# cloudwego/dynamicgo

Hardware: AMD Instinct MI355X
Metric: conv/j2t GB/s JSON in + msgs/s, 64K-batch device-resident, 1→8 MI355X (higher is better)
Workload: dtype u8; 1 GPU; C2: 65536 flat baseline.Simple messages <=256 B, seed 42; global_batch=65536, msgs_per_rank=65536, thrift_bytes_rank0=6662181, flags=1, parallelism=dp1 (one batch per rank, descriptor broadcast over -), no data-path collective, inflight=2

## Files before the change

dynamicgo_amd/build.py:

```python
import hashlib
import os
import subprocess
import sys

ROOT = os.path.dirname(os.path.dirname(os.path.abspath(__file__)))
CSRC = os.path.join(ROOT, "dynamicgo_amd", "csrc")
HIPCC = os.environ.get("HIPCC", "/opt/rocm/bin/hipcc")
ARCH = os.environ.get("DG_OFFLOAD_ARCH", "gfx950")


def _run(cmd, cwd=None):
    print("+", " ".join(cmd), flush=True)
    subprocess.run(cmd, cwd=cwd, check=True)


UNITS = ("j2t_kern_wave.hip", "j2t_kern_wave5.hip", "j2t_kern_small.hip", "j2t_kern_lds.hip", "j2t_kern_glb.hip",
         "j2t_host.hip", "j2t_pipe.hip", "t2j_kern.hip", "t2j_host.hip", "j2t_kern_flat.hip",
         "tget_kern.hip", "tget_host.hip", "cut_kern.hip", "cut_host.hip", "edit_kern.hip", "edit_host.hip",
         "kids_kern.hip", "kids_host.hip", "editm_kern.hip", "editm_host.hip")
HEADERS = ("j2t_small.h", "j2t_wave.h", "j2t_machine.h", "j2t_device.h", "j2t_fast.h", "dg_tables.h", "host_internal.h",
           "t2j_device.h", "t2j_tables.h", "j2t_flat.h", "t2j_wave.h", "tget_device.h", "cut_device.h", "edit_device.h",
           "kids_device.h", "editm_device.h")


def source_hash(extra_flags=()) -> str:
    h = hashlib.sha256()
    for f in sorted(UNITS + HEADERS):
        with open(os.path.join(CSRC, f), "rb") as fh:
            h.update(f.encode() + b"\0" + fh.read())
    for f in ("dgj2t.h", "dgj2t_defs.h", "dgj2t_desc.h"):
        with open(os.path.join(ROOT, "include", f), "rb") as fh:
            h.update(f.encode() + b"\0" + fh.read())
    h.update(repr((ARCH, COMMON_FLAGS, sorted(DEFAULT_UNIT_FLAGS.items()), tuple(extra_flags))).encode())
    return h.hexdigest()[:16]


COMMON_FLAGS = ("-O3", "-std=c++17", "-fPIC", "-ffp-contract=off", "-Wno-unused-result")
_NO_LICM = ("-mllvm", "-disable-machine-licm")
DEFAULT_UNIT_FLAGS = {"j2t_kern_flat.hip": _NO_LICM, "j2t_kern_wave.hip": _NO_LICM, "j2t_kern_wave5.hip": _NO_LICM,
                      "t2j_kern.hip": _NO_LICM}
MARK = b"dgj2t-build:"


def _deps(unit: str):
    import re
    seen, todo = [], [unit]
    while todo:
        f = todo.pop()
        if f in seen:
            continue
        seen.append(f)
        p = os.path.join(CSRC, f) if os.path.exists(os.path.join(CSRC, f)) else os.path.join(ROOT, "include", f)
        with open(p) as fh:
            for inc in re.findall(r'^\s*#\s*include\s+"([^"]+)"', fh.read(), re.M):
                todo.append(os.path.basename(inc))
    return sorted(seen)


def unit_hash(unit: str, extra_flags=()) -> str:
    h = hashlib.sha256()
    for f in _deps(unit):
        p = os.path.join(CSRC, f) if os.path.exists(os.path.join(CSRC, f)) else os.path.join(ROOT, "include", f)
        with open(p, "rb") as fh:
            h.update(f.encode() + b"\0" + fh.read())
    h.update(repr((ARCH, COMMON_FLAGS, tuple(extra_flags))).encode())
    return h.hexdigest()[:16]


def embedded_hash(path: str):
    try:
        with open(path, "rb") as fh:
            data = fh.read()
    except OSError:
        return None
    k = data.find(MARK)
    if k < 0:
        return None
    return data[k + len(MARK):k + len(MARK) + 16].decode("ascii", "replace")


def build_hip(force=False, extra_flags=(), out=None, unit_flags=None):
    out = out or os.path.join(ROOT, "dynamicgo_amd", "libdgj2t.so")
    unit_flags = unit_flags or {}
    sh = source_hash(tuple(extra_flags) + tuple(sorted((u, tuple(f)) for u, f in unit_flags.items())))
    uf0 = dict(DEFAULT_UNIT_FLAGS)
    for u, f in unit_flags.items():
        uf0[u] = tuple(uf0.get(u, ())) + tuple(f)
    unit_flags = uf0
    if not force and embedded_hash(out) == sh:
        print(f"libdgj2t.so up to date (sources {sh})", flush=True)
        return out
    objdir = os.path.join(ROOT, "build", "obj")
    os.makedirs(objdir, exist_ok=True)
    common = [HIPCC, f"--offload-arch={ARCH}", *COMMON_FLAGS, *extra_flags]
    procs, objs = [], []
    for u in UNITS:
        uf = tuple(extra_flags) + tuple(unit_flags.get(u, ()))
        uh = unit_hash(u, uf) + (sh if u == "j2t_host.hip" else "")
        o = os.path.join(objdir, u.replace(".hip", "") + "_" + uh + ".o")
        objs.append(o)
        if os.path.exists(o) and not force:
            continue
        cmd = common + list(unit_flags.get(u, ())) + ([f'-DDG_SRC_HASH="{sh}"'] if u == "j2t_host.hip" else [])
        cmd = cmd + ["-c", "-o", o + ".tmp", os.path.join(CSRC, u)]
        print("+", " ".join(cmd), flush=True)
# ... 29 lines not shown
```

dynamicgo_amd/csrc/host_internal.h:

```cpp
#pragma once
#include <hip/hip_runtime.h>

#include <stdint.h>
#include <stdlib.h>

#include <algorithm>
#include <memory>
#include <mutex>
#include <vector>

#include "../../include/dgj2t.h"
#include "../../include/dgj2t_desc.h"

__attribute__((visibility("hidden"))) int set_err(int code, const char *fmt, ...);
#define HIPCHK(x)                                                                              \
    do {                                                                                       \
        hipError_t e_ = (x);                                                                   \
        if (e_ != hipSuccess) return set_err(DG_E_HIP, "%s: %s", #x, hipGetErrorString(e_));  \
    } while (0)


template <class T, hipError_t (*FREE)(void *)>
struct ArrBase {
    T *p = nullptr;
// ... 186 lines not shown
};

struct PipeBuf;
struct PipeBufDelete {
    void operator()(PipeBuf *p) const;
};

struct dg_ctx {
    int device = 0;
    Stream stream;
    int n_cu = 0;
    Knobs knobs;
    uint32_t rr = 0;
    std::mutex mu;
    const Event *kt = nullptr;
    Event fork_ev;
    std::vector<Event> side_ev;
    std::vector<Stream> side;
    SharedWs tget;
    DevArr<uint32_t> tget_list, tget_cnt_buf;
    AltCounters tget_cnt;
    StreamOrder cut;
    DevArr<uint32_t> cut_list, cut_cnt_buf;
    AltCounters cut_cnt;
    StreamOrder edit;
    DevArr<dg_tget_rec> edit_rec;
    uint64_t edit_rec_n = 0;
    StreamOrder editm;
    DevArr<dg_tget_rec> editm_rec;
    SharedWs kids;
    DevArr<uint32_t> kids_list, kids_cnt_buf;
    AltCounters kids_cnt;
    DevArr<uint64_t> kids_sums;
    SharedWs t2j_tok;
    SharedWs t2j_deep;
    PinArr<uint8_t> h_down;
    PinArr<uint8_t> h_up;
    DevArr<uint64_t> d_pack_off;
    DevArr<uint8_t> d_pack;
    DevArr<uint8_t> d_cb;
    DevArr<uint64_t> d_aux;
    DevArr<uint64_t> d_ret;
    DevArr<uint32_t> d_out_len;
    DevArr<uint64_t> d_out_off;
    DevArr<uint8_t> d_out;
    DevArr<uint64_t> d_in_off;
    DevArr<uint8_t> d_json;
    DevArr<unsigned long long> d_stats;
    DevArr<uint64_t> d_zero;
    DevArr<uint32_t> d_pending;
    std::vector<std::unique_ptr<Scratch>> scratch;
    std::mutex pipe_mu;
    PinArr<uint8_t> h_pipe_aux, h_pipe_out;
    PinArr<uint8_t> h_pipe_ovf;
    DevArr<uint64_t> d_pipe_cur;
    std::vector<std::unique_ptr<PipeBuf, PipeBufDelete>> pipe;
    ~dg_ctx()
    {
        (void)hipSetDevice(device);
        if (stream) (void)hipStreamSynchronize(stream);
    }
};

struct Entry {
    std::unique_lock<std::mutex> lk;
    hipStream_t s = nullptr;
    int rc = DG_OK;
    Entry(dg_ctx *c, bool ok, void *stream = nullptr, const char *what = "bad args")
    {
        if (!ok) {
            rc = set_err(DG_E_INVALID, "%s", what);
            return;
        }
        lk = std::unique_lock<std::mutex>(c->mu);
        const hipError_t e = hipSetDevice(c->device);
        if (e != hipSuccess) rc = set_err(DG_E_HIP, "hipSetDevice(c->device): %s", hipGetErrorString(e));
        s = stream ? (hipStream_t)stream : (hipStream_t)c->stream;
    }
};

struct dg_desc {
    dg_ctx *ctx = nullptr;
    DevArr<uint8_t> d_blob;
    size_t len = 0;
    dg_desc_hdr hdr;
    DevArr<uint8_t> d_side;
    std::vector<uint8_t> hblob;
    size_t side_len = 0;
};

struct dg_path {
    dg_ctx *ctx;
    DevArr<uint8_t> d_blob;
    dg_path_hdr hdr;
};

struct TGetBatch {
    const uint8_t *src;
    const uint64_t *in_off;
    uint64_t n;
    dg_tget_rec *rec;
    uint64_t *val_off;
    uint32_t *val_len;
    uint64_t max_len;
};

__attribute__((visibility("hidden"))) int dg_i_path_validate(const void *blob, size_t len, dg_path_hdr &h);

__attribute__((visibility("hidden"))) int tget_launch(dg_ctx *c, const dg_path *ps, uint8_t root_type,
                                                      const TGetBatch &b, hipStream_t s);

struct HMIn {
    const dg_hm_entry *tab = nullptr;
    uint32_t n_hm = 0;
    const uint8_t *bytes = nullptr;
    const dg_cb_entry *vm = nullptr;
};

struct BatchArgs {
    const uint8_t *src = nullptr;
    const uint64_t *in_off = nullptr;
    uint64_t n = 0, flags = 0;
    uint8_t *out = nullptr;
    const uint64_t *out_off = nullptr;
    uint32_t *out_len = nullptr;
    uint64_t *ret = nullptr;
    uint32_t *pending = nullptr;
    uint64_t max_len = 0;
    HMIn hm;
    uint64_t *aux = nullptr;
};

struct HostOut {
    uint8_t *out;
    uint64_t out_cap;
    uint64_t *out_off, *out_need;
};

struct PackChain {
    const uint64_t *base_in = nullptr;
    uint64_t dst_cap = 0;
    int base_mod16 = 0;
    uint64_t *ret_dst = nullptr, *cur_out = nullptr, *ovf_out = nullptr;
    hipEvent_t pack_after = nullptr;
};

__attribute__((visibility("hidden"))) void dg_i_scratch_release(dg_ctx *c, const hipStream_t *s, int n);

__attribute__((visibility("hidden"))) int scratch_for(dg_ctx *c, hipStream_t s, Scratch **out);

__attribute__((visibility("hidden"))) int dg_i_convert_pack(dg_ctx *c, const dg_desc *d, uint32_t root,
                                                            const BatchArgs &b, uint8_t *packed, uint64_t *pack_off,
                                                            hipStream_t s, const PackChain &ch);

__attribute__((visibility("hidden"))) int dg_i_pack_scan(dg_ctx *c, hipStream_t s, const BatchArgs &b, uint8_t *d_dst,
                                                         uint64_t *d_dst_off);
```

dynamicgo_amd/csrc/j2t_flat.h:

```cpp
#pragma once
#include "j2t_small.h"

namespace dg {

constexpr uint32_t FL_G = 4;
#ifndef DG_FL_WAVES
#define DG_FL_WAVES 4
#endif
constexpr uint32_t FL_WAVES = DG_FL_WAVES;
#ifndef DG_FL_FPW
#define DG_FL_FPW 2
#endif
constexpr uint32_t FL_FPW = DG_FL_FPW;
constexpr uint32_t FL_SLOTS = FL_FPW * FL_WAVES;
constexpr uint32_t FL_MPB = 64;
constexpr uint32_t FL_LW = 9;
constexpr uint32_t FL_MAXLEN = 256;
constexpr uint32_t FL_SLOTW = FL_MAXLEN / 8;
constexpr uint32_t FL_STAGEW = FL_MPB * FL_SLOTW;
constexpr uint32_t FL_SLACKW = FL_G * FL_LW + 2;
constexpr uint32_t FL_MAXF = 24;
constexpr uint32_t FL_DESC = 16 * 1024;
#ifndef DG_FL_INLINE
#define DG_FL_INLINE 8
#endif
#ifndef DG_FL_CHUNK
#define DG_FL_CHUNK 32
#endif
constexpr uint32_t FL_INLINE = DG_FL_INLINE;
constexpr uint32_t FL_CHUNK = DG_FL_CHUNK;
constexpr uint32_t FL_MAXTASK = 320;
constexpr uint32_t FL_KEYS = 32;
constexpr uint32_t FL_NESC = 8;
#ifndef DG_FL_WPE
#define DG_FL_WPE 4
#endif

#ifndef DG_FL_DEFER_NUM
#define DG_FL_DEFER_NUM 0
#endif
#ifndef DG_FL_PERM
#define DG_FL_PERM 0
#endif
#ifndef DG_FL_REMAP
#define DG_FL_REMAP 1
#endif

#ifdef DG_FLPROF_G
#define FLG_ARG , uint64_t *flg
#define FLG_PASS , flg
#define FLG(k)                                             \
    do {                                                   \
        const uint64_t now_ = __builtin_amdgcn_s_memtime(); \
        flg[k] += now_ - flg[7];                           \
        flg[7] = now_;                                     \
    } while (0)
#else
#define FLG_ARG
#define FLG_PASS
#define FLG(k)
#endif
DGI uint32_t fl_slot(uint32_t w, uint32_t h)
{
    return DG_FL_PERM == 1 ? (h & 1 ? (h + 1) * FL_WAVES - 1 - w : h * FL_WAVES + w) : w + h * FL_WAVES;
}

#define DG_DPP(v, ctrl) ((uint32_t)__builtin_amdgcn_update_dpp(0, (int)(v), (ctrl), 0xF, 0xF, false))
DGI uint32_t g4_incl_sum(uint32_t v, uint32_t g)
{
    uint32_t t = DG_DPP(v, 0x111);
    v += g >= 1 ? t : 0u;
    t = DG_DPP(v, 0x112);
    v += g >= 2 ? t : 0u;
    return v;
}
DGI uint32_t g4_sum(uint32_t v)
{
    v += DG_DPP(v, 0xB1);
    v += DG_DPP(v, 0x4E);
    return v;
}
DGI uint32_t g4_next(uint32_t v, uint32_t g)
{
    const uint32_t t = DG_DPP(v, 0x101);
    return g < 3 ? t : 0u;
}

DGI uint32_t eq32(uint32_t w, uint32_t cc) { return zb32(w ^ cc); }

struct LSrc {
    typedef int32_t idx;
    const __attribute__((address_space(3))) uint64_t *w8;
    int32_t off0;
    int32_t n;
    DGI void init(const __attribute__((address_space(3))) uint64_t *words, int32_t off, int32_t len)
    {
        w8 = words;
        off0 = off;
        n = len;
    }
    DGI uint8_t raw(int32_t i) const
    {
        return ((const __attribute__((address_space(3))) uint8_t *)w8)[off0 + i];
    }
    DGI uint8_t at(int32_t i) const { return (uint32_t)i < (uint32_t)n ? raw(i) : 0; }
    DGI uint64_t get8(int32_t i) const
    {
        const uint32_t b = (uint32_t)(off0 + i), k = b >> 3, sh = (b & 7) << 3;
        const uint64_t lo = w8[k], hi = w8[k + 1];
        return (lo >> sh) | ((hi << 1) << (63 - sh));
    }
    DGI LSrc sub(int32_t s0, int32_t len) const
    {
        LSrc r;
        r.init(w8, off0 + s0, len);
        return r;
// ... 314 lines not shown
DGI bool body_b64(S &src, uint32_t s0, uint32_t n, bool last, O &o)
{
    typedef typename S::idx SI;
    uint32_t ip = 0;
    const uint32_t full = last && n >= 4 ? n - 4 : n;
    for (; ip + 8 <= full; ip += 8) {
        uint64_t v;
        if (!b64_8(src.get8((SI)(s0 + ip)), v)) return false;
        o.wle(v, 6);
    }
    for (; ip < full; ip += 4) {
        uint32_t v;
        if (!b64_4((uint32_t)src.get8((SI)(s0 + ip)), v)) return false;
        o.wle(v, 3);
    }
    if (last && n >= 4) {
        uint32_t w = (uint32_t)src.get8((SI)(s0 + ip));
        const uint32_t c2 = (w >> 16) & 0xFF, c3 = w >> 24;
        if (c2 == '=' && c3 != '=') return false;
        const uint32_t keep = c3 == '=' ? (c2 == '=' ? 1u : 2u) : 3u;
        if (c3 == '=') w = (w & 0x00FFFFFFu) | ((uint32_t)'A' << 24);
        if (c2 == '=') w = (w & 0xFF00FFFFu) | ((uint32_t)'A' << 16);
        uint32_t v;
        if (!b64_4(w, v)) return false;
        o.wle(v, keep);
    }
    return true;
}

template <class S, class O>
DGI uint32_t flat_write(S &src, const FField &F, const FastTabs &tb, O &o, lds_esc *E, uint32_t ne)
{
    typedef typename S::idx SI;
    if (F.kind == FV_NONE) return 1;
    bool isint = F.isint;
    int64_t iv = F.iv;
    double dv = F.dv;
    if (F.kind == FV_NUM && F.defer) {
        SI qq = (SI)F.s0;
        if (!fast_vnumber(src, qq, tb, iv, dv, isint) || (uint32_t)qq != F.s0 + F.nb) return 0;
    }
    o.wle((uint32_t)F.tt | ((uint32_t)__builtin_bswap16(F.id) << 8), 3);
    switch (F.kind) {
    case FV_BOOL: o.w8((uint8_t)iv); return 1;
    case FV_NUM:
        if (F.i16q) {
            emit_number(o, DG_T_I16, isint, iv, dv);
            emit_number(o, DG_T_BYTE, isint, iv, dv);
            return 1;
        }
        return emit_number(o, F.tt, isint, iv, dv) ? 1u : 0u;
    case FV_NUMSTR:
    case FV_STR:
        o.w32(F.kind == FV_NUMSTR ? F.nb : F.size - 7);
        if (F.esc) {
            uint32_t cur = F.s0;
            const uint32_t end = F.s0 + F.nb;
            for (uint32_t it = 0; it < FL_NESC; it++) {
                uint32_t best = 0xFFFFFFFFu;
                for (uint32_t e = 0; e < ne; e++) {
                    const uint32_t x = E[e], p = esc_pos(x);
                    if (p >= cur && p < end && p < esc_pos(best)) best = x;
                }
                if (best == 0xFFFFFFFFu) break;
                const uint32_t p = esc_pos(best);
                body_copy(src, cur, p - cur, o);
                o.wle(esc_utf8(best), esc_out(best));
                cur = p + esc_in(best);
            }
            body_copy(src, cur, end - cur, o);
            return 1;
        }
        if (F.nb > FL_INLINE) return 2;
        body_copy(src, F.s0, F.nb, o);
        return 1;
    default:
        o.w32(F.size - 7);
        if (F.nb > FL_INLINE) return 2;
        return body_b64(src, F.s0, F.nb, true, o) ? 1u : 0u;
    }
}

struct FlatParams {
    const uint8_t *blob;
    dg_desc_hdr hdr;
    uint32_t *bail_count;
    uint32_t *bail_list;
    uint32_t wrap;
    uint32_t wrap_inner;
    uint64_t wrap_ok;
};

#ifdef DG_FLPROF
#define FLP_DECL uint64_t flp_t = __builtin_amdgcn_s_memtime(); uint64_t flp[8] = {0, 0, 0, 0, 0, 0, 0, 0};
#define FLP(k)                                              \
    do {                                                    \
        const uint64_t now_ = __builtin_amdgcn_s_memtime(); \
        flp[k] += now_ - flp_t;                             \
        flp_t = now_;                                       \
    } while (0)
#define FLP_END()                                                                        \
    do {                                                                                 \
        if ((threadIdx.x & 63) == 0 && (blockIdx.x & 31) == 0)                           \
            for (int k_ = 0; k_ < 8; k_++) atomicAdd(&P.stats[2 + k_], (unsigned long long)flp[k_]); \
    } while (0)
#else
#define FLP_DECL
#define FLP(k)
#define FLP_END()
#endif
#ifdef DG_FLPROF_F
#define FLF_DECL uint64_t flf[12] = {0, 0, 0, 0, 0, 0, 0, 0, 0, 0, 0, 0};
#define FLF_T0() const uint64_t flf_t0 = __builtin_amdgcn_s_memtime()
#define FLF_ADD(k) do { if ((k) < 12) flf[k] += __builtin_amdgcn_s_memtime() - flf_t0; } while (0)
#define FLF_END()                                                                         \
    do {                                                                                  \
        if ((threadIdx.x & 63) == 0 && (blockIdx.x & 31) == 0)                            \
            for (int k_ = 0; k_ < 12; k_++) atomicAdd(&P.stats[2 + k_], (unsigned long long)flf[k_]); \
    } while (0)
#else
#define FLF_DECL
#define FLF_T0()
#define FLF_ADD(k)
#define FLF_END()
#endif

struct FlatLds {
    uint64_t in[FL_STAGEW + FL_SLACKW];
    uint64_t task[FL_MAXTASK];
    uint64_t oa[FL_MPB];
    uint32_t cap[FL_MPB];
    uint32_t ok[FL_MPB];
    uint32_t n[FL_MPB];
    uint32_t lw[FL_MPB];
    uint32_t oc[FL_MPB];
    uint32_t nfq[FL_MPB];
    uint32_t plo[FL_MPB], phi[FL_MPB];
    uint32_t big[FL_MPB];
    uint32_t nbytes[FL_MPB];
    uint32_t wid[FL_MPB];
    uint32_t nesc[FL_MPB];
    uint32_t esc[FL_MPB * FL_NESC];
    uint64_t kw[2 * FL_KEYS];
    uint32_t km[FL_KEYS];
    uint32_t fkm[FL_SLOTS];
    uint32_t sep[FL_MAXF * FL_MPB];
    uint16_t col[FL_MAXF * FL_MPB];
    uint16_t size[2 * FL_SLOTS * FL_MPB];
    uint32_t fseen[FL_MPB];
    uint32_t rounds, ntask, tgrab, noremap;
    uint8_t *a_out;
    uint64_t *a_ret;
    uint32_t *a_out_len, *a_bail_count, *a_bail_list;
    uint32_t a_nb, a_wrap;
    uint64_t p10u[20];
    double p10d[23];
    uint64_t pw[EL_WN];
};

template <int V>
__global__ __launch_bounds__(64 * FL_WAVES) __attribute__((amdgpu_waves_per_eu(DG_FL_WPE))) void j2t_flat_kernel(
    Params P, FlatParams S)
{
    __shared__ __attribute__((aligned(16))) FlatLds L;
    extern __shared__ __attribute__((aligned(16))) uint64_t s_fdesc[];
    FLP_DECL
    FLF_DECL
    const uint32_t tid = threadIdx.x, lane = tid & 63, wave = tid >> 6;
    const uint64_t b0 = (uint64_t)blockIdx.x * FL_MPB;
    const uint64_t b1 = b0 + FL_MPB < P.n ? b0 + FL_MPB : P.n;

    const uint64_t lo = P.in_off[b0], hi = P.in_off[b1];
    const uint64_t base = lo & ~15ull;
    const bool staged = hi - base <= (uint64_t)FL_STAGEW * 8;
    if (staged) {
        const uint4 *gs = (const uint4 *)(P.json + base);
        uint4 *ls = (uint4 *)L.in;
        const uint32_t nw = (uint32_t)((hi - base + 15) >> 4);
        constexpr uint32_t NT = 64 * FL_WAVES;
        static_assert(FL_STAGEW * 8 / 16 <= 4 * NT, "four 16-byte loads per thread cover the stage");
        if (nw) {
            const uint32_t l = nw - 1;
            const uint4 v0 = gs[min(tid, l)], v1 = gs[min(tid + NT, l)], v2 = gs[min(tid + 2 * NT, l)],
                        v3 = gs[min(tid + 3 * NT, l)];
            if (tid < nw) ls[tid] = v0;
            if (tid + NT < nw) ls[tid + NT] = v1;
            if (tid + 2 * NT < nw) ls[tid + 2 * NT] = v2;
            if (tid + 3 * NT < nw) ls[tid + 3 * NT] = v3;
        }
    }
    {
        const uint4 *gd = (const uint4 *)S.blob;
        uint4 *ld = (uint4 *)s_fdesc;
        for (uint32_t k = tid; k < (S.hdr.total_len + 15) / 16; k += 64 * FL_WAVES) ld[k] = gd[k];
    }
    if (tid < 20) {
        uint64_t v = 1;
        for (uint32_t k = 0; k < tid; k++) v *= 10;
        L.p10u[tid] = v;
    }
    if (tid < 23) L.p10d[tid] = P10[tid];
    el_window_fill(L.pw, tid);
    if (tid == 0) {
        L.rounds = 0;
        L.ntask = 0;
        L.tgrab = 0;
        L.noremap = 0;
        L.a_out = P.out;
        L.a_ret = P.ret;
        L.a_out_len = P.out_len;
        L.a_bail_count = S.bail_count;
        L.a_bail_list = S.bail_list;
        L.a_nb = (uint32_t)(b1 - b0);
        L.a_wrap = S.wrap;
    }
    if (tid < FL_MPB) {
        uint32_t ok = 0, n = 0, lw = 0, big = 0, cap = 0;
        uint64_t oa = 0;
        const uint64_t i = b0 + tid;
        if (i < b1) {
            const uint64_t a = P.in_off[i], b = P.in_off[i + 1];
            const uint64_t n64 = b - a;
            oa = P.out_off[i];
            cap = (uint32_t)min(P.out_off[i + 1] - oa, (uint64_t)0xFFFFFFFFu);
            const bool tobig = P.big_list && (n64 > P.big_max || n64 > FL_MAXLEN);
            list_big_w(P, tobig, i, n64);
            if (tobig) {
                big = 1;
            } else if (n64 > 0 && n64 <= FL_MAXLEN) {
                n = (uint32_t)n64;
                if (staged) {
                    ok = 1;
                    lw = (uint32_t)(((a - base) >> 3) << 3) | (uint32_t)(a & 7);
                } else {
                    ok = 1;
                    lw = (tid * FL_SLOTW) << 3;
                }
            }
        }
        L.ok[tid] = ok;
        L.n[tid] = n;
        L.lw[tid] = lw;
        L.big[tid] = big;
        L.oa[tid] = oa;
        L.cap[tid] = cap;
        L.plo[tid] = 0;
        L.phi[tid] = 0;
        L.oc[tid] = 0;
        L.nfq[tid] = 0;
        L.nesc[tid] = 0;
        L.fseen[tid] = 0;
    }
    if (tid < FL_SLOTS * FL_MPB / 4) ((uint32_t *)(void *)L.task)[tid] = 0xFFFFFFFFu;
    __syncthreads();
    const uint32_t g = tid & 3, m1 = tid >> 2;
    if (!staged) {
        if (tid < FL_G * FL_MPB && L.ok[m1]) {
            const uint64_t a = P.in_off[b0 + m1];
            const uint32_t nw = (L.n[m1] + 7) >> 3, sh = (uint32_t)(a & 7) << 3;
            const glb_u64 *gsrc = (const glb_u64 *)(const void *)P.json + (a >> 3);
            constexpr uint32_t NWL = FL_MAXLEN / 8 / FL_G;
            uint64_t lo[NWL], hi[NWL];
#pragma unroll
            for (uint32_t j = 0; j < NWL; j++) {
                const uint32_t w = g + FL_G * j;
                lo[j] = gsrc[min(w, nw)];
                hi[j] = gsrc[min(w + 1, nw)];
            }
#pragma unroll
            for (uint32_t j = 0; j < NWL; j++) {
                const uint32_t w = g + FL_G * j;
                if (w < nw) L.in[(L.lw[m1] >> 3) + w] = sh ? (lo[j] >> sh) | (hi[j] << (64 - sh)) : lo[j];
            }
        }
        __syncthreads();
    }
    FLP(0);
#if defined(DG_FL_STOP) && DG_FL_STOP == 9
    return;
#endif
    const auto D = desc_view<3>((const __attribute__((address_space(3))) uint8_t *)(void *)s_fdesc, S.hdr);
    const FastTabs tb{(const __attribute__((address_space(3))) uint64_t *)(void *)L.p10u, (lds_f64 *)(void *)L.p10d,
                      (const __attribute__((address_space(3))) uint64_t *)(void *)L.pw};
    const dg_type rt = ldrec(&D.T[S.wrap ? S.wrap_inner : P.root]);
    const dg_struct sd = ldrec(&D.S[rt.st]);
    const uint32_t nk = sd.name_mask + 1 <= FL_KEYS ? sd.name_mask + 1 : 0u;
    if (tid < nk) {
        const dg_name nm = ldrec(&D.N[sd.name_begin + tid]);
        uint32_t mt = 0xFF000000u;
        uint64_t w0 = 0, w1 = 0;
        if (nm.field != DG_NONE && nm.key_len <= 16) {
            const __attribute__((address_space(3))) uint64_t *pk = (decltype(&D.R[0]))(&D.P[nm.key_off]);
            w0 = nm.key_len ? pk[0] : 0ull;
            w1 = nm.key_len > 8 ? pk[1] : 0ull;
            mt = nm.field | (nm.key_len << 24);
        }
        L.km[tid] = mt;
        L.kw[2 * tid] = w0;
        L.kw[2 * tid + 1] = w1;
    }
    if (tid >= 64 && tid < 64 + FL_SLOTS) {
        const uint32_t j = tid - 64;
        uint32_t len = 0xFF;
        if (j < sd.n_fields) {
            const dg_field f = ldrec(&D.F[sd.field_begin + j]);
            if (f.flags & DG_FF_ALIAS_SELF) len = f.key_len;
        }
        L.fkm[j] = len;
    }
    if (S.wrap) {
        if (tid < FL_MPB) {
            uint32_t wid = 0;
            if (L.ok[tid]) {
                const uint32_t n = L.n[tid], lwa = L.lw[tid];
                LSrc src;
                src.init((const __attribute__((address_space(3))) uint64_t *)(void *)&L.in[lwa >> 3], (int32_t)(lwa & 7),
                         (int32_t)n);
                uint32_t p = skip_ws(src, 0);
                bool ok = p < n && src.raw((int32_t)p) == '{';
                p = ok ? skip_ws(src, p + 1) : p;
                ok = ok && p < n && src.raw((int32_t)p) == '"';
                const uint32_t k0 = p + 1;
                uint32_t q = k0;
                while (ok && q < n && src.raw((int32_t)q) != '"') {
                    if (src.raw((int32_t)q) == '\\') ok = false;
                    q++;
                }
                ok = ok && q < n;
                const uint32_t kn = q - k0;
                p = ok ? skip_ws(src, q + 1) : p;
                ok = ok && p < n && src.raw((int32_t)p) == ':';
                p = ok ? skip_ws(src, p + 1) : p;
                ok = ok && p < n && src.raw((int32_t)p) == '{';
                uint32_t e = n;
                while (ok && e > p && isspace_(src.raw((int32_t)(e - 1)))) e--;
                ok = ok && e > p + 1 && src.raw((int32_t)(e - 1)) == '}';
                uint32_t ic = e - 1;
                while (ok && ic > p && isspace_(src.raw((int32_t)(ic - 1)))) ic--;
                ok = ok && ic > p + 1 && src.raw((int32_t)(ic - 1)) == '}';
                if (ok) {
                    const dg_struct rs = ldrec(&D.S[ldrec(&D.T[P.root]).st]);
                    const int32_t fi = fl_lookup(D, rs, src, k0, kn);
                    const uint32_t k = (uint32_t)fi - rs.field_begin;
                    ok = fi >= 0 && k < 64 && ((S.wrap_ok >> k) & 1);
                    if (ok) {
                        wid = 0x10000u | ldrec(&D.F[fi]).id;
                        L.lw[tid] = lwa + p;
                        L.n[tid] = ic - p;
                        L.oa[tid] += 3;
                        L.cap[tid] = L.cap[tid] > 4 ? L.cap[tid] - 4 : 0u;
                    }
                }
                if (!ok) L.ok[tid] = 0;
            }
            L.wid[tid] = wid;
        }
        __syncthreads();
    }

    if (tid < FL_G * FL_MPB) {
        const bool on = L.ok[m1] != 0;
        const uint32_t n = L.n[m1], lwa = L.lw[m1], a7 = lwa & 7, lw = lwa >> 3;
        const int32_t nv0 = on ? (int32_t)n - 64 * (int32_t)g : 0;
        const uint32_t nv = nv0 <= 0 ? 0u : nv0 >= 64 ? 64u : (uint32_t)nv0;
        const uint64_t vmask = nv >= 64 ? ~0ull : (1ull << nv) - 1;
        uint32_t d[18];
// ... 314 lines not shown
        if (wave == 0) L.nbytes[mm] = nbytes;
#ifdef DG_FLPROF_G
        if (lane == 0 && (blockIdx.x & 31) == 0)
            for (int k_ = 0; k_ < 6; k_++) atomicAdd(&P.stats[2 + k_], (unsigned long long)flg[k_]);
#endif
    }
    FLP(6);
    {
        const uint32_t nt = min(L.ntask, FL_MAXTASK);
        for (;;) {
            uint32_t t0 = 0;
            if (lane == 0) t0 = atomicAdd(&L.tgrab, 64u);
            t0 = (uint32_t)__builtin_amdgcn_readfirstlane((int)t0);
            if (t0 >= nt) break;
            const uint32_t t = t0 + lane;
            const uint64_t tk = t < nt ? L.task[t] : ~0ull;
            if (tk == ~0ull) continue;
            const uint32_t m = (uint32_t)tk & 63, s0 = (uint32_t)(tk >> 8) & 0xFFF, cn = (uint32_t)(tk >> 20) & 0xFFF;
            const uint32_t lwa = L.lw[m];
            LSrc src;
            src.init((const __attribute__((address_space(3))) uint64_t *)(void *)&L.in[lwa >> 3], (int32_t)(lwa & 7), (int32_t)L.n[m]);
            WOut o;
            o.init((gu8 *)(void *)(L.a_out + L.oa[m] + (uint32_t)(tk >> 32)));
#ifdef DG_FL_ABL_NOSTORE
            o.dry = true;
#endif
            bool cok = true;
            if ((tk >> 6) & 1) cok = body_b64(src, s0, cn, ((tk >> 7) & 1) != 0, o);
            else body_copy(src, s0, cn, o);
            o.finish();
            if (!cok) L.ok[m] = 0;
        }
    }
    __syncthreads();
    FLP(7);

    if (tid < FL_MPB) {
        const uint32_t m = tid;
        const uint64_t i = (uint64_t)blockIdx.x * FL_MPB + m;
        if (m < L.a_nb) {
            const uint32_t len = L.nbytes[m] + 1;
            const uint32_t wid = L.a_wrap ? L.wid[m] : 0u;
            bool good = L.ok[m] && len <= L.cap[m];
            if (good) {
                const uint64_t present = (uint64_t)L.plo[m] | ((uint64_t)L.phi[m] << 32);
                uint64_t bits = D.R[sd.req_begin] & ~present;
                const uint64_t flag = P.flag;
                while (bits) {
                    const uint32_t kk = (uint32_t)__builtin_ctzll(bits);
                    bits &= bits - 1;
                    const dg_field f = ldrec(&D.F[sd.field_begin + kk]);
                    if (f.flags & DG_FF_REQUEST_BASE) continue;
                    if (f.required == DG_REQ_REQUIRED || ((flag & DG_F_WRITE_DEFAULT) && f.required == DG_REQ_DEFAULT) ||
                        ((flag & DG_F_WRITE_OPTIONAL) && f.required == DG_REQ_OPTIONAL)) {
                        good = false;
                        break;
                    }
                }
            }
            if (good && wid) {
                gu8 *o = (gu8 *)(void *)L.a_out + L.oa[m];
                o[-3] = DG_T_STRUCT;
                o[-2] = (uint8_t)(wid >> 8);
                o[-1] = (uint8_t)wid;
                o[len - 1] = 0;
                o[len] = 0;
                L.a_ret[i] = 0;
                L.a_out_len[i] = len + 4;
            } else if (good) {
                ((gu8 *)(void *)L.a_out)[L.oa[m] + len - 1] = 0;
                L.a_ret[i] = 0;
                L.a_out_len[i] = len;
            } else if (!L.big[m]) {
                const uint32_t qq = atomicAdd(L.a_bail_count, 1u);
                L.a_bail_list[qq] = (uint32_t)i;
            }
        }
    }
    FLP_END();
    FLF_END();
}

void launch_flat_kernel(dim3 grid, hipStream_t s, const Params &P, const FlatParams &S);

}
```

dynamicgo_amd/csrc/j2t_host.hip:

```cpp
#include <hip/hip_runtime.h>

#include <stdarg.h>
#include <stdio.h>
#include <stdlib.h>
#include <string.h>

#include <algorithm>
#include <mutex>
#include <vector>

#include "j2t_flat.h"
#include "host_internal.h"

using namespace dg;

static thread_local char g_err[512];
int set_err(int code, const char *fmt, ...)
{
    va_list ap;
    va_start(ap, fmt);
    vsnprintf(g_err, sizeof g_err, fmt, ap);
    va_end(ap);
    return code;
}
// ... 73 lines not shown
    if (!strcmp(name, "small_mpw")) return &K.small_mpw;
    if (!strcmp(name, "list_blocks")) return &K.list_blocks;
    if (!strcmp(name, "t2j_spread")) return &K.t2j_spread;
    if (!strcmp(name, "t2j_wave_min")) return &K.t2j_wave_min;
    if (!strcmp(name, "t2j_overlap")) return &K.t2j_overlap;
    if (!strcmp(name, "flat_wrap")) return &K.flat_wrap;
    if (!strcmp(name, "tget_spread")) return &K.tget_spread;
    if (!strcmp(name, "cut_wave_min")) return &K.cut_wave_min;
    if (!strcmp(name, "edit_wave_min")) return &K.edit_wave_min;
    if (!strcmp(name, "edit_reuse_rec")) return &K.edit_reuse_rec;
    if (!strcmp(name, "edit_lanes")) return &K.edit_lanes;
    if (!strcmp(name, "kids_wide_min")) return &K.kids_wide_min;
    if (!strcmp(name, "kids_no_scan")) return &K.kids_no_scan;
    return nullptr;
}

extern "C" {

const char *dg_last_error(void) { return g_err; }

const char *dg_build_info(void) { return g_build_info; }

int dg_ctx_create(int device, dg_ctx **out)
{
    if (!out) return set_err(DG_E_INVALID, "null out");
    int ndev = 0;
    HIPCHK(hipGetDeviceCount(&ndev));
    if (device < 0 || device >= ndev) return set_err(DG_E_INVALID, "device %d out of range (%d)", device, ndev);
    HIPCHK(hipSetDevice(device));
    std::unique_ptr<dg_ctx> c(new dg_ctx());
    c->device = device;
    HIPCHK(c->stream.create(hipStreamDefault));
    int rc;
    if ((rc = c->d_pending.alloc(4)) || (rc = c->d_zero.alloc(2))) return rc;
    HIPCHK(hipMemset(c->d_zero, 0, 16));
    if ((rc = c->d_stats.alloc(16))) return rc;
    HIPCHK(hipMemset(c->d_stats, 0, 16 * 8));
    HIPCHK(hipDeviceSynchronize());
    HIPCHK(hipDeviceGetAttribute(&c->n_cu, hipDeviceAttributeMultiprocessorCount, device));
    static const struct { const char *env; const char *name; } envk[] = {
        {"DG_FLAT", "flat"}, {"DG_WAVE_MIN", "wave_min"}, {"DG_WAVE_OCC", "wave_occ"},
        {"DG_SMALL_MPW", "small_mpw"}, {"DG_LIST_BLOCKS", "list_blocks"}, {"DG_T2J_SPREAD", "t2j_spread"},
        {"DG_T2J_WAVE_MIN", "t2j_wave_min"}, {"DG_T2J_OVERLAP", "t2j_overlap"}, {"DG_FLAT_WRAP", "flat_wrap"},
        {"DG_TGET_SPREAD", "tget_spread"}, {"DG_CUT_WAVE_MIN", "cut_wave_min"},
        {"DG_EDIT_WAVE_MIN", "edit_wave_min"}, {"DG_EDIT_LANES", "edit_lanes"},
        {"DG_KIDS_WIDE_MIN", "kids_wide_min"}};
    for (const auto &e : envk) {
        const char *v = getenv(e.env);
        if (v && *v) *knob_ref(c.get(), e.name) = strtoll(v, nullptr, 10);
    }
    *out = c.release();
    return DG_OK;
}

int dg_ctx_set_knob(dg_ctx *c, const char *name, int64_t value)
{
    if (!c || !name) return set_err(DG_E_INVALID, "null ctx/name");
    std::lock_guard<std::mutex> g(c->mu);
    int64_t *k = knob_ref(c, name);
    if (!k) return set_err(DG_E_INVALID, "unknown knob '%s'", name);
    *k = value;
    return DG_OK;
}

int dg_ctx_get_knob(dg_ctx *c, const char *name, int64_t *value)
{
    if (!c || !name || !value) return set_err(DG_E_INVALID, "bad args");
    std::lock_guard<std::mutex> g(c->mu);
    int64_t *k = knob_ref(c, name);
    if (!k) return set_err(DG_E_INVALID, "unknown knob '%s'", name);
    *value = *k;
    return DG_OK;
}

void dg_ctx_destroy(dg_ctx *c) { delete c; }

void *dg_ctx_stream(dg_ctx *c) { return c ? (void *)(hipStream_t)c->stream : nullptr; }

static int desc_finish(dg_ctx *c, const dg_desc_hdr &h, DevArr<uint8_t> &d_blob, size_t len, const void *host_blob,
                       dg_desc **out)
{
    if (h.magic != DG_DESC_MAGIC || h.version < 1 || h.version > DG_DESC_VERSION || h.total_len > len)
        return set_err(DG_E_DESC, "bad descriptor blob header");
    dg_desc *d = new dg_desc();
    d->ctx = c;
    d->d_blob = std::move(d_blob);
    d->len = len;
    d->hdr = h;
    d->hblob.assign((const uint8_t *)host_blob, (const uint8_t *)host_blob + h.total_len);
    *out = d;
    return DG_OK;
}

static bool flat_root(const dg_desc *d, uint32_t root, uint64_t flags)
{
    const dg_desc_hdr &h = d->hdr;
    if (d->hblob.size() < h.total_len || h.version < 2 || h.total_len > FL_DESC || root >= h.n_types) return false;
    const uint8_t *b = d->hblob.data();
    const dg_type *T = (const dg_type *)(b + h.off_types);
    if (T[root].ttype != DG_T_STRUCT) return false;
    const dg_struct &sd = ((const dg_struct *)(b + h.off_structs))[T[root].st];
    if (sd.req_words != 1 || ((flags & DG_F_ENABLE_HM) && (sd.flags & DG_SF_HTTP_MAPPING))) return false;
    const dg_field *F = (const dg_field *)(b + h.off_fields);
    for (uint32_t k = 0; k < sd.n_fields; k++) {
        switch (T[F[sd.field_begin + k].type].ttype) {
        case DG_T_BOOL: case DG_T_BYTE: case DG_T_I16: case DG_T_I32: case DG_T_I64: case DG_T_DOUBLE: case DG_T_STRING:
            break;
        default:
            return false;
        }
    }
    return true;
}

static uint64_t wrap_root(const dg_desc *d, uint32_t root, uint64_t flags, uint32_t *inner)
{
    const dg_desc_hdr &h = d->hdr;
    if (d->hblob.size() < h.total_len || h.version < 2 || h.total_len > FL_DESC || root >= h.n_types) return 0;
    const uint8_t *b = d->hblob.data();
    const dg_type *T = (const dg_type *)(b + h.off_types);
    if (T[root].ttype != DG_T_STRUCT) return 0;
    const dg_struct &rs = ((const dg_struct *)(b + h.off_structs))[T[root].st];
    if (rs.req_words != 1 || rs.n_fields > 64 || ((flags & DG_F_ENABLE_HM) && (rs.flags & DG_SF_HTTP_MAPPING))) return 0;
    const dg_field *F = (const dg_field *)(b + h.off_fields);
    const uint64_t req = ((const uint64_t *)(b + h.off_reqwords))[rs.req_begin];
    uint32_t w = DG_NONE;
    for (uint32_t k = 0; k < rs.n_fields && w == DG_NONE; k++) {
        const uint32_t t = F[rs.field_begin + k].type;
        if (T[t].ttype == DG_T_STRUCT && flat_root(d, t, flags)) w = t;
    }
    if (w == DG_NONE) return 0;
    uint64_t ok = 0;
    for (uint32_t k = 0; k < rs.n_fields; k++) {
        const dg_field &f = F[rs.field_begin + k];
        if (f.type != w || ((flags & DG_F_ENABLE_VM) && f.vm != DG_VM_NONE) ||
            ((f.flags & DG_FF_REQUEST_BASE) && (flags & DG_F_NO_WRITE_BASE)))
            continue;
        bool fine = true;
        for (uint32_t j = 0; j < rs.n_fields && fine; j++) {
            if (j == k || !((req >> j) & 1)) continue;
            const dg_field &g = F[rs.field_begin + j];
            if (g.flags & DG_FF_REQUEST_BASE) continue;
            if ((flags & DG_F_TRACE_BACK) || g.required == DG_REQ_REQUIRED ||
                ((flags & DG_F_WRITE_DEFAULT) && g.required == DG_REQ_DEFAULT) ||
                ((flags & DG_F_WRITE_OPTIONAL) && g.required == DG_REQ_OPTIONAL))
                fine = false;
        }
        if (fine) ok |= 1ull << k;
    }
    *inner = w;
    return ok;
}

int dg_desc_create(dg_ctx *c, const void *blob, size_t len, dg_desc **out)
{
    if (!c || !blob || !out || len < sizeof(dg_desc_hdr)) return set_err(DG_E_INVALID, "bad args");
    dg_desc_hdr h;
    memcpy(&h, blob, sizeof h);
    if (h.magic != DG_DESC_MAGIC || h.total_len > len) return set_err(DG_E_DESC, "bad descriptor blob");
    HIPCHK(hipSetDevice(c->device));
    DevArr<uint8_t> d_blob;
    if (int rc = d_blob.alloc(len)) return rc;
    HIPCHK(hipMemcpy(d_blob, blob, len, hipMemcpyHostToDevice));
    return desc_finish(c, h, d_blob, len, blob, out);
}

int dg_desc_create_device(dg_ctx *c, const void *d_src, size_t len, dg_desc **out)
{
    if (!c || !d_src || !out || len < sizeof(dg_desc_hdr)) return set_err(DG_E_INVALID, "bad args");
// ... 73 lines not shown
    auto mark = [&](int i) {
        if (c->kt) (void)hipEventRecord(c->kt[i], s);
    };
    flags &= ~(DG_F_NO_WAVE_PATH | DG_F_FLAT_PATH | DG_F_NO_FLAT_PATH);
    uint32_t *const cnt = x->counts;
    Params P;
    P.root = root;
    P.json = b.src;
    P.in_off = b.in_off;
    P.n = n;
    P.flag = flags;
    P.list = nullptr;
    P.list_count = nullptr;
    P.reset2 = nullptr;
    P.big_list = nullptr;
    P.big_count = nullptr;
    P.big_max = 0;
    P.huge_count = nullptr;
    P.huge_min = WV_HUGE_MIN;
    P.hm_tab = b.hm.tab;
    P.hm_bytes = b.hm.bytes;
    P.n_hm = b.hm.n_hm;
    P.ans_tab = b.hm.vm;
    P.out = b.out;
    P.out_off = b.out_off;
    P.out_len = b.out_len;
    P.ret = b.ret;
    P.pending = b.pending;
    P.deep_count = cnt + CNT_DEEP;
    P.deep_list = x->deep_list;
    P.ws = x->ws_fast;
    P.ws_stride = FAST_WS_STRIDE;
    P.keycap = WS_KEYCAP;
    P.reqcap = WS_REQCAP;
    P.fast = d->hdr.version >= 2 && (flags & ~FAST_FLAGS) == 0;
    P.stats = c->d_stats;
    const uint64_t blocks = (n + LANE_BLOCK - 1) / LANE_BLOCK;
    DeepParams DP;
    DP.ws = x->ws_deep;
    DP.ws_stride = DEEP_WS_STRIDE;
    DP.keycap = DEEP_KEYCAP;
    DP.reqcap = DEEP_REQCAP;
    DP.done = cnt + CNT_DEEP_DONE;
    DP.blob = d->d_blob;
    DP.hdr = d->hdr;
    const uint64_t big_max = (uint64_t)K.wave_min;
    const bool may_be_long = max_len == 0 || max_len > big_max;
    const bool wave = P.fast && !no_wave && d->hdr.total_len <= WV_DESC && d->hdr.total_len <= DESC_LDS_BYTES &&
                      may_be_long;
    auto lane_launch = [&](uint64_t grid, const Params &Q) {
        if (d->hdr.total_len <= DESC_LDS_BYTES) launch_lane_kernel_lds(dim3((uint32_t)grid), s, Q, DP);
        else launch_lane_kernel_glb(dim3((uint32_t)grid), s, Q, DP);
    };
    const int mpw = (int)K.small_mpw;
    const bool small = P.fast && !no_wave && mpw > 0 && d->hdr.total_len <= SM_DESC;
    if (!small && !wave) {
        mark(0);
        lane_launch(blocks, P);
        mark(1);
        mark(2);
        mark(3);
        HIPCHK(hipGetLastError());
        return DG_OK;
    }
    if ((rc = x->grow(x->bail_list, n))) return rc;
    if ((rc = x->grow(x->big_list, n))) return rc;
    const bool wave_stage = small ? may_be_long : true;
    Params P1 = P;
    if (wave_stage) {
        P1.big_list = x->big_list;
        P1.big_count = cnt + CNT_BIG;
        P1.big_max = big_max;
        P1.huge_count = cnt + CNT_HUGE;
    }
    uint32_t inner = DG_NONE;
    const uint64_t wrap_ok = (small && K.flat_wrap != 0 && !no_flat && !flat_root(d, root, flags))
                                 ? wrap_root(d, root, flags, &inner)
                                 : 0;
    mark(0);
    if (!small) {
        lane_launch(blocks, P1);
    } else if ((use_flat && flat_root(d, root, flags)) || wrap_ok) {
        FlatParams FP;
        FP.blob = d->d_blob;
        FP.hdr = d->hdr;
        FP.bail_count = cnt + CNT_BAIL;
        FP.bail_list = x->bail_list;
        FP.wrap = wrap_ok ? 1u : 0u;
        FP.wrap_inner = wrap_ok ? inner : 0u;
        FP.wrap_ok = wrap_ok;
        launch_flat_kernel(dim3((uint32_t)((n + FL_MPB - 1) / FL_MPB)), s, P1, FP);
    } else {
        SmallParams S;
        S.blob = d->d_blob;
        S.hdr = d->hdr;
        S.bail_count = cnt + CNT_BAIL;
        S.bail_list = x->bail_list;
        const uint64_t mpb = (uint64_t)SM_WAVES * (uint64_t)(mpw >= 64 ? 64 : mpw == 16 ? 16 : 32);
        launch_small_kernel(mpw, dim3((uint32_t)((n + mpb - 1) / mpb)), s, P1, S);
    }
    HIPCHK(hipGetLastError());
    mark(1);
    if (wave_stage) {
        WaveParams W;
        W.blob = d->d_blob;
        W.hdr = d->hdr;
        W.bail_count = cnt + CNT_BAIL;
        W.bail_list = x->bail_list;
        W.list = x->big_list;
        W.list_count = cnt + CNT_BIG;
        W.huge_count = cnt + CNT_HUGE;
        W.list_cap = n;
        W.ws = x->ws_wave;
        W.queue = cnt + CNT_WAVEQ;
        const bool wave5 = K.wave_occ == 5;
        const uint64_t bpc = wave5 ? WV5_BLOCKS_PER_CU : WV_BLOCKS_PER_CU;
        const dim3 wgrid((uint32_t)std::min<uint64_t>((n + WV_WAVES - 1) / WV_WAVES, (uint64_t)c->n_cu * bpc));
        if (wave5) launch_wave_kernel5(wgrid, s, P, W);
        else launch_wave_kernel(wgrid, s, P, W);
        HIPCHK(hipGetLastError());
    }
    mark(2);
    Params P3 = P;
    P3.list = x->bail_list;
    P3.list_count = cnt + CNT_BAIL;
    P3.reset2 = cnt + CNT_BIG;
    if (!small) P3.fast = 0;
    const uint64_t cap = small ? (uint64_t)std::max<int64_t>(1, K.list_blocks) : 32;
    lane_launch(std::min<uint64_t>(blocks, cap), P3);
    mark(3);
    HIPCHK(hipGetLastError());
    return DG_OK;
}

static int launch(dg_ctx *c, const dg_desc *d, uint32_t root, const BatchArgs &b, hipStream_t s)
{
    if (b.n == 0) return DG_OK;
    if (root >= d->hdr.n_types) return set_err(DG_E_INVALID, "root type %u out of range", root);
    Scratch *x;
    int rc = scratch_for(c, s, &x);
    if (rc) return rc;
    rc = enqueue(c, x, d, root, b, s);
    if (rc) (void)hipMemsetAsync(x->counts, 0, DG_J2T_COUNTS_BYTES, s);
    HIPCHK(x->publish(s));
    return rc;
}

int dg_j2t_batch_device(dg_ctx *c, const dg_desc *d, uint32_t root, const uint8_t *d_json, const uint64_t *d_in_off,
                        uint64_t n, uint64_t flags, uint8_t *d_out, const uint64_t *d_out_off, uint32_t *d_out_len,
                        uint64_t *d_ret, uint32_t *d_pending, void *stream)
{
    Entry g(c, c && d, stream, "null ctx/desc");
    if (g.rc) return g.rc;
    const BatchArgs b{d_json, d_in_off, n, flags, d_out, d_out_off, d_out_len, d_ret, d_pending};
    return launch(c, d, root, b, g.s);
}

int dg_j2t_batch_device_ml(dg_ctx *c, const dg_desc *d, uint32_t root, const uint8_t *d_json, const uint64_t *d_in_off,
                           uint64_t n, uint64_t flags, uint8_t *d_out, const uint64_t *d_out_off, uint32_t *d_out_len,
                           uint64_t *d_ret, uint32_t *d_pending, void *stream, uint64_t max_len)
{
    Entry g(c, c && d, stream, "null ctx/desc");
    if (g.rc) return g.rc;
    const BatchArgs b{d_json, d_in_off, n, flags, d_out, d_out_off, d_out_len, d_ret, d_pending, max_len};
    return launch(c, d, root, b, g.s);
}

// ... 462 lines not shown
```

dynamicgo_amd/csrc/j2t_kern_flat.hip:

```cpp
#include "j2t_flat.h"

namespace dg {
void launch_flat_kernel(dim3 grid, hipStream_t s, const Params &P, const FlatParams &S)
{
    const uint32_t shmem = (S.hdr.total_len + 15) & ~15u;
    hipLaunchKernelGGL(j2t_flat_kernel<0>, grid, dim3(64 * FL_WAVES), shmem, s, P, S);
}
}
```

Baseline: 430.2 GB/s.

## Prebuild descriptor+table image on host and restructure flat-kernel prologue

```diff
diff --git a/dynamicgo_amd/build.py b/dynamicgo_amd/build.py
--- a/dynamicgo_amd/build.py
+++ b/dynamicgo_amd/build.py
@@ -17,10 +17,10 @@
 UNITS = ("j2t_kern_wave.hip", "j2t_kern_wave5.hip", "j2t_kern_small.hip", "j2t_kern_lds.hip", "j2t_kern_glb.hip",
          "j2t_host.hip", "j2t_pipe.hip", "t2j_kern.hip", "t2j_host.hip", "j2t_kern_flat.hip",
          "tget_kern.hip", "tget_host.hip", "cut_kern.hip", "cut_host.hip", "edit_kern.hip", "edit_host.hip",
-         "kids_kern.hip", "kids_host.hip", "editm_kern.hip", "editm_host.hip")
+         "kids_kern.hip", "kids_host.hip", "editm_kern.hip", "editm_host.hip", "flat_image.hip")
 HEADERS = ("j2t_small.h", "j2t_wave.h", "j2t_machine.h", "j2t_device.h", "j2t_fast.h", "dg_tables.h", "host_internal.h",
            "t2j_device.h", "t2j_tables.h", "j2t_flat.h", "t2j_wave.h", "tget_device.h", "cut_device.h", "edit_device.h",
-           "kids_device.h", "editm_device.h")
+           "kids_device.h", "editm_device.h", "flat_image.h")
 
 
 def source_hash(extra_flags=()) -> str:
diff --git a/dynamicgo_amd/csrc/flat_image.h b/dynamicgo_amd/csrc/flat_image.h
--- /dev/null
+++ b/dynamicgo_amd/csrc/flat_image.h
@@ -0,0 +1,33 @@
+#pragma once
+#include <stdint.h>
+#include <string.h>
+
+namespace dg {
+
+constexpr int FLI_WLO = -40;
+constexpr int FLI_WN = 64;
+constexpr uint32_t FLI_NP10U = 20, FLI_NP10D = 23;
+constexpr uint32_t FLI_P10U = 0;
+constexpr uint32_t FLI_P10D = FLI_P10U + 8 * FLI_NP10U;
+constexpr uint32_t FLI_PW = FLI_P10D + 8 * FLI_NP10D;
+constexpr uint32_t FLI_TABS = (FLI_PW + 8 * FLI_WN + 15) & ~15u;
+
+static const double FLI_P10D_VALUES[FLI_NP10D] = {1e0,  1e1,  1e2,  1e3,  1e4,  1e5,  1e6,  1e7,  1e8,  1e9,  1e10, 1e11,
+                                                  1e12, 1e13, 1e14, 1e15, 1e16, 1e17, 1e18, 1e19, 1e20, 1e21, 1e22};
+
+constexpr uint32_t fli_blob16(uint32_t total_len) { return (total_len + 15) & ~15u; }
+constexpr uint32_t fli_len(uint32_t total_len) { return fli_blob16(total_len) + FLI_TABS; }
+
+inline void fli_build(const uint8_t *blob, uint32_t total_len, const uint64_t (*pw_hi)[2], uint8_t *img)
+{
+    const uint32_t b16 = fli_blob16(total_len);
+    memset(img, 0, fli_len(total_len));
+    memcpy(img, blob, total_len);
+    uint8_t *t = img + b16;
+    uint64_t v = 1;
+    for (uint32_t k = 0; k < FLI_NP10U; k++, v *= 10) memcpy(t + FLI_P10U + 8 * k, &v, 8);
+    memcpy(t + FLI_P10D, FLI_P10D_VALUES, sizeof FLI_P10D_VALUES);
+    for (int k = 0; k < FLI_WN; k++) memcpy(t + FLI_PW + 8 * k, &pw_hi[FLI_WLO + 348 + k][1], 8);
+}
+
+}
diff --git a/dynamicgo_amd/csrc/flat_image.hip b/dynamicgo_amd/csrc/flat_image.hip
--- /dev/null
+++ b/dynamicgo_amd/csrc/flat_image.hip
@@ -0,0 +1,15 @@
+#include <stdint.h>
+
+#undef __device__
+#define __device__
+#undef __constant__
+#define __constant__
+#include "dg_tables.h"
+#include "flat_image.h"
+
+namespace dg {
+void flat_image_build(const uint8_t *blob, uint32_t total_len, uint8_t *img)
+{
+    fli_build(blob, total_len, DG_POW10_M128, img);
+}
+}
diff --git a/dynamicgo_amd/csrc/host_internal.h b/dynamicgo_amd/csrc/host_internal.h
--- a/dynamicgo_amd/csrc/host_internal.h
+++ b/dynamicgo_amd/csrc/host_internal.h
@@ -292,6 +292,7 @@
 struct dg_desc {
     dg_ctx *ctx = nullptr;
     DevArr<uint8_t> d_blob;
+    DevArr<uint8_t> d_flat;
     size_t len = 0;
     dg_desc_hdr hdr;
     DevArr<uint8_t> d_side;
diff --git a/dynamicgo_amd/csrc/j2t_flat.h b/dynamicgo_amd/csrc/j2t_flat.h
--- a/dynamicgo_amd/csrc/j2t_flat.h
+++ b/dynamicgo_amd/csrc/j2t_flat.h
@@ -1,4 +1,5 @@
 #pragma once
+#include "flat_image.h"
 #include "j2t_small.h"
 
 namespace dg {
@@ -32,6 +33,9 @@
 constexpr uint32_t FL_MAXTASK = 320;
 constexpr uint32_t FL_KEYS = 32;
 constexpr uint32_t FL_NESC = 8;
+static_assert(FLI_WLO == EL_WLO && FLI_WN == EL_WN, "the image's window is FastTabs' window");
+constexpr uint32_t FL_FMAPW = FL_SLOTS * FL_MPB / 8;
+static_assert(FL_MAXTASK >= FL_FMAPW + FL_MPB, "the task area holds the field map and, behind it, an unstaged block's offsets");
 #ifndef DG_FL_WPE
 #define DG_FL_WPE 4
 #endif
@@ -512,7 +516,7 @@
 }
 
 struct FlatParams {
-    const uint8_t *blob;
+    const uint8_t *img;
     dg_desc_hdr hdr;
     uint32_t *bail_count;
     uint32_t *bail_list;
@@ -583,10 +587,8 @@
     uint64_t *a_ret;
     uint32_t *a_out_len, *a_bail_count, *a_bail_list;
     uint32_t a_nb, a_wrap;
-    uint64_t p10u[20];
-    double p10d[23];
-    uint64_t pw[EL_WN];
 };
+static_assert(sizeof(FlatLds) % 16 == 0, "the image behind FlatLds starts 16-byte aligned");
 
 template <int V>
 __global__ __launch_bounds__(64 * FL_WAVES) __attribute__((amdgpu_waves_per_eu(DG_FL_WPE))) void j2t_flat_kernel(
@@ -599,38 +601,27 @@
     const uint32_t tid = threadIdx.x, lane = tid & 63, wave = tid >> 6;
     const uint64_t b0 = (uint64_t)blockIdx.x * FL_MPB;
     const uint64_t b1 = b0 + FL_MPB < P.n ? b0 + FL_MPB : P.n;
-
-    const uint64_t lo = P.in_off[b0], hi = P.in_off[b1];
+    const uint32_t nb = (uint32_t)(b1 - b0);
+    constexpr uint32_t NT = 64 * FL_WAVES;
+    static_assert(FL_WAVES >= 4, "the prologue gives waves 0..3 a part each");
+
+    const uint32_t blob16 = fli_blob16(S.hdr.total_len);
+    const uint32_t ni = (blob16 + FLI_TABS) >> 4;
+    const uint4 *gi = (const uint4 *)S.img;
+    const uint4 i0 = gi[min(tid, ni - 1)], i1 = gi[min(tid + NT, ni - 1)];
+    const uint64_t *po = (wave & 1) ? P.out_off : P.in_off;
+    const uint64_t ov = po[b0 + min(lane, nb)];
+    const uint64_t lo = P.in_off[b0], hi = P.in_off[b1], oend = P.out_off[b1];
     const uint64_t base = lo & ~15ull;
     const bool staged = hi - base <= (uint64_t)FL_STAGEW * 8;
-    if (staged) {
-        const uint4 *gs = (const uint4 *)(P.json + base);
-        uint4 *ls = (uint4 *)L.in;
-        const uint32_t nw = (uint32_t)((hi - base + 15) >> 4);
-        constexpr uint32_t NT = 64 * FL_WAVES;
-        static_assert(FL_STAGEW * 8 / 16 <= 4 * NT, "four 16-byte loads per thread cover the stage");
-        if (nw) {
-            const uint32_t l = nw - 1;
-            const uint4 v0 = gs[min(tid, l)], v1 = gs[min(tid + NT, l)], v2 = gs[min(tid + 2 * NT, l)],
-                        v3 = gs[min(tid + 3 * NT, l)];
-            if (tid < nw) ls[tid] = v0;
-            if (tid + NT < nw) ls[tid + NT] = v1;
-            if (tid + 2 * NT < nw) ls[tid + 2 * NT] = v2;
-            if (tid + 3 * NT < nw) ls[tid + 3 * NT] = v3;
-        }
-    }
-    {
-        const uint4 *gd = (const uint4 *)S.blob;
-        uint4 *ld = (uint4 *)s_fdesc;
-        for (uint32_t k = tid; k < (S.hdr.total_len + 15) / 16; k += 64 * FL_WAVES) ld[k] = gd[k];
-    }
-    if (tid < 20) {
-        uint64_t v = 1;
-        for (uint32_t k = 0; k < tid; k++) v *= 10;
-        L.p10u[tid] = v;
-    }
-    if (tid < 23) L.p10d[tid] = P10[tid];
-    el_window_fill(L.pw, tid);
+    const uint32_t nw = staged ? (uint32_t)((hi - base + 15) >> 4) : 0u;
+    static_assert(FL_STAGEW * 8 / 16 <= 4 * NT, "four 16-byte loads per thread cover the stage");
+    const uint4 *gs = (const uint4 *)(P.json + base);
+    const uint32_t l = nw ? nw - 1 : 0u;
+    const uint4 v0 = gs[min(tid, l)], v1 = gs[min(tid + NT, l)], v2 = gs[min(tid + 2 * NT, l)],
+                v3 = gs[min(tid + 3 * NT, l)];
+    const uint64_t onx = __shfl_down(ov, 1);
+    const uint64_t nx = lane == 63 ? ((wave & 1) ? oend : hi) : onx;
     if (tid == 0) {
         L.rounds = 0;
         L.ntask = 0;
@@ -641,52 +632,59 @@
         L.a_out_len = P.out_len;
         L.a_bail_count = S.bail_count;
         L.a_bail_list = S.bail_list;
-        L.a_nb = (uint32_t)(b1 - b0);
+        L.a_nb = nb;
         L.a_wrap = S.wrap;
     }
-    if (tid < FL_MPB) {
-        uint32_t ok = 0, n = 0, lw = 0, big = 0, cap = 0;
-        uint64_t oa = 0;
-        const uint64_t i = b0 + tid;
-        if (i < b1) {
-            const uint64_t a = P.in_off[i], b = P.in_off[i + 1];
-            const uint64_t n64 = b - a;
-            oa = P.out_off[i];
-            cap = (uint32_t)min(P.out_off[i + 1] - oa, (uint64_t)0xFFFFFFFFu);
-            const bool tobig = P.big_list && (n64 > P.big_max || n64 > FL_MAXLEN);
-            list_big_w(P, tobig, i, n64);
-            if (tobig) {
-                big = 1;
-            } else if (n64 > 0 && n64 <= FL_MAXLEN) {
-                n = (uint32_t)n64;
-                if (staged) {
-                    ok = 1;
-                    lw = (uint32_t)(((a - base) >> 3) << 3) | (uint32_t)(a & 7);
-                } else {
-                    ok = 1;
-                    lw = (tid * FL_SLOTW) << 3;
-                }
-            }
-        }
-        L.ok[tid] = ok;
-        L.n[tid] = n;
-        L.lw[tid] = lw;
-        L.big[tid] = big;
-        L.oa[tid] = oa;
-        L.cap[tid] = cap;
-        L.plo[tid] = 0;
-        L.phi[tid] = 0;
-        L.oc[tid] = 0;
-        L.nfq[tid] = 0;
-        L.nesc[tid] = 0;
-        L.fseen[tid] = 0;
-    }
-    if (tid < FL_SLOTS * FL_MPB / 4) ((uint32_t *)(void *)L.task)[tid] = 0xFFFFFFFFu;
+    const uint32_t wv = (uint32_t)__builtin_amdgcn_readfirstlane((int)wave);
+    if (wv == 0) {
+        uint32_t ok = 0, n = 0, lw = 0, big = 0;
+        const bool live = lane < nb;
+        const uint64_t a = ov, n64 = live ? nx - a : 0;
+        const bool tobig = live && P.big_list && (n64 > P.big_max || n64 > FL_MAXLEN);
+        list_big_w(P, tobig, b0 + lane, n64);
+        if (tobig) {
+            big = 1;
+        } else if (n64 > 0 && n64 <= FL_MAXLEN) {
+            n = (uint32_t)n64;
+            ok = 1;
+            if (staged) lw = (uint32_t)(((a - base) >> 3) << 3) | (uint32_t)(a & 7);
+            else lw = (lane * FL_SLOTW) << 3;
+        }
+        L.ok[lane] = ok;
+        L.n[lane] = n;
+        L.lw[lane] = lw;
+        L.big[lane] = big;
+        if (!staged) L.task[FL_FMAPW + lane] = a;
+    } else if (wv == 1) {
+        const bool live = lane < nb;
+        L.oa[lane] = live ? ov : 0;
+        L.cap[lane] = live ? (uint32_t)min(nx - ov, (uint64_t)0xFFFFFFFFu) : 0u;
+    } else if (wv == 2) {
+        L.plo[lane] = 0;
+        L.phi[lane] = 0;
+        L.oc[lane] = 0;
+        L.nfq[lane] = 0;
+        L.nesc[lane] = 0;
+        L.fseen[lane] = 0;
+    } else if (wv == 3) {
+        for (uint32_t k = lane; k < FL_FMAPW; k += 64) L.task[k] = ~0ull;
+    }
+    {
+        uint4 *ls = (uint4 *)L.in;
+        if (tid < nw) ls[tid] = v0;
+        if (tid + NT < nw) ls[tid + NT] = v1;
+        if (tid + 2 * NT < nw) ls[tid + 2 * NT] = v2;
+        if (tid + 3 * NT < nw) ls[tid + 3 * NT] = v3;
+        uint4 *li = (uint4 *)s_fdesc;
+        if (tid < ni) li[tid] = i0;
+        if (tid + NT < ni) li[tid + NT] = i1;
+        for (uint32_t k = tid + 2 * NT; k < ni; k += NT) li[k] = gi[k];
+    }
     __syncthreads();
     const uint32_t g = tid & 3, m1 = tid >> 2;
     if (!staged) {
         if (tid < FL_G * FL_MPB && L.ok[m1]) {
-            const uint64_t a = P.in_off[b0 + m1];
+            const uint64_t a = L.task[FL_FMAPW + m1];
             const uint32_t nw = (L.n[m1] + 7) >> 3, sh = (uint32_t)(a & 7) << 3;
             const glb_u64 *gsrc = (const glb_u64 *)(const void *)P.json + (a >> 3);
             constexpr uint32_t NWL = FL_MAXLEN / 8 / FL_G;
@@ -710,8 +708,10 @@
     return;
 #endif
     const auto D = desc_view<3>((const __attribute__((address_space(3))) uint8_t *)(void *)s_fdesc, S.hdr);
-    const FastTabs tb{(const __attribute__((address_space(3))) uint64_t *)(void *)L.p10u, (lds_f64 *)(void *)L.p10d,
-                      (const __attribute__((address_space(3))) uint64_t *)(void *)L.pw};
+    const __attribute__((address_space(3))) uint8_t *tabs =
+        (const __attribute__((address_space(3))) uint8_t *)(void *)s_fdesc + blob16;
+    const FastTabs tb{(const __attribute__((address_space(3))) uint64_t *)(tabs + FLI_P10U), (lds_f64 *)(tabs + FLI_P10D),
+                      (const __attribute__((address_space(3))) uint64_t *)(tabs + FLI_PW)};
     const dg_type rt = ldrec(&D.T[S.wrap ? S.wrap_inner : P.root]);
     const dg_struct sd = ldrec(&D.S[rt.st]);
     const uint32_t nk = sd.name_mask + 1 <= FL_KEYS ? sd.name_mask + 1 : 0u;
@@ -1192,5 +1192,6 @@
 }
 
 void launch_flat_kernel(dim3 grid, hipStream_t s, const Params &P, const FlatParams &S);
-
-}
+void flat_image_build(const uint8_t *blob, uint32_t total_len, uint8_t *img);
+
+}
diff --git a/dynamicgo_amd/csrc/j2t_host.hip b/dynamicgo_amd/csrc/j2t_host.hip
--- a/dynamicgo_amd/csrc/j2t_host.hip
+++ b/dynamicgo_amd/csrc/j2t_host.hip
@@ -179,9 +179,17 @@
 {
     if (h.magic != DG_DESC_MAGIC || h.version < 1 || h.version > DG_DESC_VERSION || h.total_len > len)
         return set_err(DG_E_DESC, "bad descriptor blob header");
+    DevArr<uint8_t> d_flat;
+    if (h.version >= 2 && h.total_len <= FL_DESC) {
+        std::vector<uint8_t> img(fli_len(h.total_len));
+        flat_image_build((const uint8_t *)host_blob, h.total_len, img.data());
+        if (int rc = d_flat.alloc(img.size())) return rc;
+        HIPCHK(hipMemcpy(d_flat, img.data(), img.size(), hipMemcpyHostToDevice));
+    }
     dg_desc *d = new dg_desc();
     d->ctx = c;
     d->d_blob = std::move(d_blob);
+    d->d_flat = std::move(d_flat);
     d->len = len;
     d->hdr = h;
     d->hblob.assign((const uint8_t *)host_blob, (const uint8_t *)host_blob + h.total_len);
@@ -421,7 +429,7 @@
         lane_launch(blocks, P1);
     } else if ((use_flat && flat_root(d, root, flags)) || wrap_ok) {
         FlatParams FP;
-        FP.blob = d->d_blob;
+        FP.img = d->d_flat;
         FP.hdr = d->hdr;
         FP.bail_count = cnt + CNT_BAIL;
         FP.bail_list = x->bail_list;
diff --git a/dynamicgo_amd/csrc/j2t_kern_flat.hip b/dynamicgo_amd/csrc/j2t_kern_flat.hip
--- a/dynamicgo_amd/csrc/j2t_kern_flat.hip
+++ b/dynamicgo_amd/csrc/j2t_kern_flat.hip
@@ -3,7 +3,7 @@
 namespace dg {
 void launch_flat_kernel(dim3 grid, hipStream_t s, const Params &P, const FlatParams &S)
 {
-    const uint32_t shmem = (S.hdr.total_len + 15) & ~15u;
+    const uint32_t shmem = fli_len(S.hdr.total_len);
     hipLaunchKernelGGL(j2t_flat_kernel<0>, grid, dim3(64 * FL_WAVES), shmem, s, P, S);
 }
 }
```

Result: faster. 457.3 GB/s (median of 6 runs) (+6.3%).
